# ZhengkunTian/Speech-Tranformer-Pytorch

Hardware: AMD Instinct MI355X
Metric: frames/sec/step (80-d fbank, 6+6L d256) at 1/2/4/8 MI355X vs CPU ref (higher is better)
Workload: dtype bf16; 1 GPU; BASELINE config 2: 6+6L d256 h4 dff1024 V4337, 80-d fbank, global B=32 split 32 per GPU (strong scaling, SURVEY 8e), T<=1000 (24060 valid frames on rank 0), L<=50; fwd+CE+bwd+clip+Adam (rate 0: weights held), dropout off; global_batch=32, parallelism=dp1, launch=hipGraph replay of the whole step, wire=fp32, dp_bucket_mb=8, nccl_algo=default, nccl_proto=default

## Files before the change

speech-tranformer-pytorch_amd/csrc/st_attn.hip:

```cpp
#include "st_attn_common.cuh"

int st_attn64_fwd_launch(hipStream_t stream, const void* args, int grid_x, int drop, int kpre);
int st_attn_xs_fwd_launch(hipStream_t stream, const void* args, int grid_x, int drop, const void* f1, const void* self);
void st_attn_xs_self_args(void* out, const void* Q, const void* K, const void* V, int ld, void* O, void* Ores, int ldo,
                          float* lse, const unsigned* drop_seed, unsigned drop_salt, int drop_thresh, float drop_scale);
int st_attn_xs_self_args_size();
void st_attn_xs_f1_args(void* out, const void* A, int lda, const void* R, int ldr, const void* wfrag, int n_blocks,
                        int next_blocks, float eps, const float* bo, const float* g0, const float* be0, void* out0,
                        void* xhat0, float* rstd0, const float* bq, void* Qout, int ldq);
int st_attn_xs_f1_args_size();
int st_attn_xs_tile_rows();
int st_attn_bwd64_launch(hipStream_t stream, const void* a, const void* ak, int n_q, int n_k, int drop);

namespace {

template <int DK, bool DROP, int KS, bool PS>
__global__ __launch_bounds__(256, (KS > 1 || DK > 64) ? 1 : 2) void attn_fwd_kernel(AttnArgs a) {
  using G = TileGeo<DK, TILE * KS>;
  constexpr int NT = DK / 16;
  constexpr int ND = DK / 32;
  constexpr int ROWS = TILE * KS, QROWS = WG_ROWS / KS;
  __shared__ __attribute__((aligned(16))) bf16 smem[4 * G::E];

  int b, h, tile;
// ... 500 lines not shown
  static const int n = [] {
    int dev = 0, cus = 0;
    if (hipGetDevice(&dev) != hipSuccess || hipDeviceGetAttribute(&cus, hipDeviceAttributeMultiprocessorCount, dev) != hipSuccess || cus <= 0) cus = 256;
    return cus;
  }();
  return n;
}
long long xsplit_bytes(int items, int xs, int d_k) { return (long long)XS_TICKETS * 4 + (long long)items * xs * 64 * d_k * 4; }

int plan(AttnArgs& a, const int* work, int n_work, int B, int H, int max_rows, int wg_rows = WG_ROWS) {
  a.work = work;
  a.H = H;
  a.tiles_max = (max_rows + wg_rows - 1) / wg_rows;
  return (work ? n_work : B * a.tiles_max) * H;
}

int attn_impl() {
  static const int v = [] { const char* e = getenv("ST_ATTN_IMPL"); return e ? atoi(e) : 0; }();
  return v;
}

struct AttnEnv {
  bool fwd64_off, xs_off;
  int bwd64;
};
AttnEnv read_attn_env() {
  auto off = [](const char* name) { const char* e = getenv(name); return e && e[0] == '0'; };
  const char* b = getenv("ST_ATTN_BWD64");
  return {off("ST_ATTN_FWD64"), off("ST_ATTN_XS"), (b && b[0] == '0') ? 1 : (b && b[0] == 'e') ? 2 : 0};
}
AttnEnv& attn_env() {
  static AttnEnv e = read_attn_env();
  return e;
}

bool fwd_long64(int d_k, int max_q, int max_k, int causal) {
  return d_k == 64 && !causal && max_q > 128 && attn_impl() != 1 && !attn_env().fwd64_off;
}

bool bwd_long64(int d_k, int max_q, int max_k, int causal, bool drop) {
  if (!(d_k == 64 && !causal && max_q > 128 && max_k > 128 && attn_impl() != 1)) return false;
  const int mode = attn_env().bwd64;
  return mode == 0 || (mode == 2 && !drop);
}

bool fwd_xs(int d_k, int max_q, int max_k, int causal) {
  return d_k == 64 && key_split(max_q, max_k, causal) && attn_impl() != 1 && !attn_env().xs_off;
}

}

extern "C" int st_env_refresh(void) {
  attn_env() = read_attn_env();
  return 0;
}

extern "C" int st_attn_tile_rows(int which, int d_k, int max_q, int max_k, int causal) {
  if (which == 0 && fwd_xs(d_k, max_q, max_k, causal)) return st_attn_xs_tile_rows();
  return WG_ROWS;
}

extern "C" int st_attn_fwd(hipStream_t stream, const void* Q, int ldq, const void* K, int ldk, const void* V, int ldv,
                           void* O, int ldo, void* Ores, float* lse, const int* q_off, const int* q_len, const int* k_off,
                           const int* k_len, int B, int H, int d_k, int max_q, int max_k, int q_rows_total, int causal,
                           float scale, const int* work, int n_work, const unsigned* drop_seed, unsigned drop_salt,
                           int drop_thresh, float drop_scale, int k_prescaled) {
  if (B <= 0 || H <= 0 || max_q <= 0 || (work && n_work <= 0)) return 0;
  int rc = check_common(d_k, ldq, ldk, ldv);
  if (rc) return rc;
  if (ldo & 7) return -3;
  if (B > 32767) return -4;
  AttnArgs a = {};
  a.Q = (const bf16*)Q; a.ldq = ldq; a.K = (const bf16*)K; a.ldk = ldk; a.V = (const bf16*)V; a.ldv = ldv;
  a.O = (bf16*)O; a.ldo = ldo; a.Ores = (bf16*)Ores; a.lse = lse; a.q_off = q_off; a.q_len = q_len; a.k_off = k_off; a.k_len = k_len;
  a.q_rows_total = q_rows_total; a.causal = causal; set_score_scales(a, scale, k_prescaled);
  const bool drop = set_drop(a, drop_seed, drop_salt, drop_thresh, drop_scale);
  a.psplit = (Ores != nullptr && max_q <= 64) ? 1 : 0;
  if (fwd_long64(d_k, max_q, max_k, causal)) {
    dim3 grid(plan(a, work, n_work, B, H, max_q));
    return st_attn64_fwd_launch(stream, &a, (int)grid.x, drop ? 1 : 0, k_prescaled ? 1 : 0);
  }
  const bool ks2 = key_split(max_q, max_k, causal);
  if (fwd_xs(d_k, max_q, max_k, causal))
    return st_attn_xs_fwd_launch(stream, &a, plan(a, work, n_work, B, H, max_q, st_attn_xs_tile_rows()), drop ? 1 : 0, nullptr, nullptr);
  dim3 grid(plan(a, work, n_work, B, H, max_q)), block(256);
#define ST_FWD(DKK, DR) \
  do { if (ks2 && a.psplit) hipLaunchKernelGGL((attn_fwd_kernel<DKK, DR, 2, true>), grid, block, 0, stream, a); \
       else if (ks2) hipLaunchKernelGGL((attn_fwd_kernel<DKK, DR, 2, false>), grid, block, 0, stream, a); \
       else if (a.psplit) hipLaunchKernelGGL((attn_fwd_kernel<DKK, DR, 1, true>), grid, block, 0, stream, a); \
       else hipLaunchKernelGGL((attn_fwd_kernel<DKK, DR, 1, false>), grid, block, 0, stream, a); } while (0)
  if (d_k == 64 && !drop) ST_FWD(64, false);
  else if (d_k == 64) ST_FWD(64, true);
  else if (d_k == 128 && !drop) ST_FWD(128, false);
  else if (d_k == 128) ST_FWD(128, true);
  else if (!drop) ST_FWD(32, false);
  else ST_FWD(32, true);
#undef ST_FWD
  ST_CHECK_LAUNCH();
  return 0;
}

extern "C" int st_attn_f1_applicable(int d_model, int d_k, int max_q, int max_k) {
  return (d_model == 256 && fwd_xs(d_k, max_q, max_k, 0)) ? 1 : 0;
}

namespace {
// ... 145 lines not shown
```

speech-tranformer-pytorch_amd/csrc/st_common.cuh:

```cuda
#pragma once

#ifdef ST_MERGE_FENCE
#define ST_PUBLISH_FENCE() __builtin_amdgcn_fence(__ATOMIC_RELEASE, "agent")
#define ST_MERGER_FENCE() __builtin_amdgcn_fence(__ATOMIC_ACQUIRE, "agent")
#else
#define ST_PUBLISH_FENCE() __builtin_amdgcn_fence(__ATOMIC_RELEASE, "wavefront")
#define ST_MERGER_FENCE() ((void)0)
#endif
#include <hip/hip_runtime.h>
#include <stdint.h>
#include "st_hip.h"

typedef __bf16 bf16;
typedef __bf16 bf16x8 __attribute__((ext_vector_type(8)));
typedef __bf16 bf16x4 __attribute__((ext_vector_type(4)));
typedef __bf16 bf16x2 __attribute__((ext_vector_type(2)));
typedef float f32x16 __attribute__((ext_vector_type(16)));
typedef float f32x4 __attribute__((ext_vector_type(4)));
typedef float f32x2 __attribute__((ext_vector_type(2)));

#define ST_WAVE 64
#define ST_LDS __attribute__((address_space(3)))

#define ST_CHECK_LAUNCH()                         \
  do {                                            \
    hipError_t e__ = hipGetLastError();           \
    if (e__ != hipSuccess) return (int)e__;       \
  } while (0)

__device__ __forceinline__ f32x16 mfma32(bf16x8 a, bf16x8 b, f32x16 c) {
  return __builtin_amdgcn_mfma_f32_32x32x16_bf16(a, b, c, 0, 0, 0);
}

__device__ __forceinline__ f32x16 zero16() {
  f32x16 z;
#pragma unroll
  for (int i = 0; i < 16; ++i) z[i] = 0.f;
  return z;
}

__device__ __forceinline__ bf16x8 zero_bf8() {
  bf16x8 z;
#pragma unroll
  for (int i = 0; i < 8; ++i) z[i] = (bf16)0.f;
  return z;
}

__device__ __forceinline__ int acc_row(int r, int hi) { return (r & 3) + 8 * (r >> 2) + 4 * hi; }

__device__ __forceinline__ bf16x8 gload8(const bf16* p, bool ok) {
  if (ok) return *reinterpret_cast<const bf16x8*>(p);
  return zero_bf8();
}

__device__ __forceinline__ bf16x8 frag_nat(const bf16* tile, int stride, int row, int c0) {
  return *reinterpret_cast<const bf16x8*>(tile + row * stride + c0);
}

__device__ __forceinline__ bf16x8 frag_tr(const bf16* tile, int stride, int row0, int ca, int cb) {
  const int l = threadIdx.x & 63;
  const int t = l & 15;
  const int colblk = ((l >> 4) & 1) * 16;
  const bf16* pa = tile + (ca + (t >> 2)) * stride + row0 + colblk + 4 * (t & 3);
  const bf16* pb = tile + (cb + (t >> 2)) * stride + row0 + colblk + 4 * (t & 3);
  bf16x4 lo = __builtin_amdgcn_ds_read_tr16_b64_v4bf16((ST_LDS bf16x4*)(pa));
  bf16x4 hi = __builtin_amdgcn_ds_read_tr16_b64_v4bf16((ST_LDS bf16x4*)(pb));
  bf16x8 f;
  f[0] = lo[0]; f[1] = lo[1]; f[2] = lo[2]; f[3] = lo[3];
  f[4] = hi[0]; f[5] = hi[1]; f[6] = hi[2]; f[7] = hi[3];
  return f;
}

__device__ __forceinline__ bf16x8 pack_acc8(const f32x16& a, int r0) {
  bf16x8 f;
#pragma unroll
// ... 68 lines not shown
```

speech-tranformer-pytorch_amd/csrc/st_gemm_sym.hip:

```cpp
#include "st_common.cuh"

#ifndef ST_GEMM_SC1
#define ST_GEMM_SC1 0
#endif
namespace {

#ifndef ST_GEMM_BK
#define ST_GEMM_BK 64
#endif
#ifndef ST_GEMM_OCC
#define ST_GEMM_OCC 2
#endif
constexpr int BK = ST_GEMM_BK;
constexpr int NS = BK + 8;
constexpr int CS_CM = 128;
constexpr int TILE_E = (128 * NS > BK * CS_CM) ? 128 * NS : BK * CS_CM;
constexpr int CH = BK / 16;
constexpr int CPR = BK / 8;

__device__ __attribute__((aligned(16))) float g_zero_f32[4];

enum Epi { EPI_BF16 = 0, EPI_BF16_RELU = 1, EPI_F32 = 2, EPI_BF16_MASK = 3, EPI_BF16_ADD = 4, EPI_F32_ATOMIC = 5,
           EPI_F32_ATOMIC_T = 6, EPI_BF16_DELTA = 7 };

// ... 468 lines not shown
}
}

extern "C" int st_wgrad_group(hipStream_t stream, int n, const void* const* X, const int* ldx, const void* const* dY,
                              const int* lddy, float* const* dW, const int* lddw, float* const* db, const int* tokens,
                              const int* K_in, const int* N_out, const int* splits) {
  for (int base = 0; base < n; base += GROUP_MAX) {
    GroupArgs g;
    g.n = 0;
    g.first[0] = 0;
    for (int q = base; q < n && q < base + GROUP_MAX; ++q) {
      if (tokens[q] <= 0 || K_in[q] <= 0 || N_out[q] <= 0) continue;
      if ((ldx[q] & 7) || (lddy[q] & 7) || (N_out[q] & 3)) return -1;
      if (ldx[q] < ((K_in[q] + 7) & ~7) || lddy[q] < ((N_out[q] + 7) & ~7)) return -3;
      GemmArgs a;
      a.M = K_in[q]; a.N = N_out[q]; a.Kc = tokens[q];
      plan_splits(a, splits[q] < 1 ? 1 : splits[q]);
      const int grid = a.splits * a.tiles_i * a.tiles_j;
      GroupProblem& p = g.p[g.n];
      p.X = (const bf16*)X[q]; p.ldx = ldx[q]; p.Y = (const bf16*)dY[q]; p.ldy = lddy[q]; p.D = dW[q]; p.ldd = lddw[q];
      p.bias = db ? db[q] : nullptr; p.M = a.M; p.N = a.N; p.Kc = a.Kc; p.c_per_split = a.c_per_split;
      p.tiles_i = a.tiles_i; p.tiles_j = a.tiles_j; p.splits = a.splits;
      g.first[g.n + 1] = g.first[g.n] + grid;
      ++g.n;
    }
    if (g.n == 0) continue;
    hipLaunchKernelGGL(gemm_wgrad_group_kernel, dim3(g.first[g.n]), dim3(256), 0, stream, g);
    ST_CHECK_LAUNCH();
  }
  return 0;
}

namespace {
int gemm_impl(hipStream_t stream, int x_cmajor, int y_cmajor, const void* X, int ldx, const void* Y,
              int ldy, void* D, int ldd, int M, int N, int Kc, float* bias, const void* aux,
              int ldaux, int epi, int splits, const unsigned* drop_seed, unsigned drop_salt,
              int drop_thresh, float drop_scale, int y_block_rows, long y_block_stride,
              long bias_block_stride, const void* aux2, void* split_work = nullptr, long long split_bytes = 0, int cs_lo = 0,
              int cs_hi = 0, float cs = 1.f) {
  if (M <= 0 || N <= 0 || Kc <= 0) return 0;
  int yseg_shift = 31;
  if (y_block_rows > 0) {
    if (y_block_rows < 128 || (y_block_rows & (y_block_rows - 1)) || x_cmajor || (y_block_stride & 7) ||
        (bias_block_stride & 3)) return -7;
    if (epi == EPI_F32_ATOMIC || epi == EPI_F32_ATOMIC_T || epi == EPI_BF16_DELTA) return -7;
    yseg_shift = __builtin_ctz(y_block_rows);
  }
  if ((ldx & 7) || (ldy & 7) || (N & 3) || epi < 0 || epi > 7) return -1;
  if (x_cmajor && !y_cmajor) return -2;
  if ((x_cmajor && ldx < ((M + 7) & ~7)) || (y_cmajor && ldy < ((N + 7) & ~7))) return -3;
  if (epi != EPI_F32 && epi != EPI_F32_ATOMIC && epi != EPI_F32_ATOMIC_T && ((ldd & 7) || (N & 7))) return -4;
  if ((epi == EPI_BF16_MASK || epi == EPI_BF16_ADD || epi == EPI_BF16_DELTA) && (ldaux & 7)) return -5;
  if (epi == EPI_BF16_DELTA && (!bias || !aux || (splits != 32 && splits != 64 && splits != 128) || (N % splits))) return -6;
  GemmArgs a;
  a.head_dim = epi == EPI_BF16_DELTA ? splits : 0;
  if (splits < 1) splits = 1;
  if (epi != EPI_F32_ATOMIC && epi != EPI_F32_ATOMIC_T && !(epi == EPI_BF16 && split_work)) splits = 1;
  a.split_ws = nullptr; a.split_tickets = nullptr;
  a.cs_lo = cs_lo; a.cs_hi = cs_hi; a.cs = cs;
  a.X = (const bf16*)X; a.ldx = ldx; a.Y = (const bf16*)Y; a.ldy = ldy; a.D = D; a.ldd = ldd;
  a.M = M; a.N = N; a.Kc = Kc; a.bias = bias; a.aux = (const bf16*)aux; a.ldaux = ldaux;
  a.aux2 = epi == EPI_BF16_DELTA ? (const bf16*)aux2 : nullptr;
  a.yseg_shift = yseg_shift;
  a.yseg_extra = y_block_rows > 0 ? y_block_stride - (long)y_block_rows * ldy : 0;
  a.bias_extra = y_block_rows > 0 ? bias_block_stride - (long)y_block_rows : 0;
  const bool drop = epi == EPI_BF16_RELU && drop_seed != nullptr && drop_thresh > 0;
  a.drop.seed = drop ? drop_seed : nullptr; a.drop.salt = drop_salt; a.drop.thresh = drop ? drop_thresh : 0;
  a.drop.scale = (drop || epi == EPI_BF16_MASK) && drop_scale > 0.f ? drop_scale : 1.f;
  dim3 grid(plan_splits(a, splits));
  if (epi == EPI_BF16 && a.splits > 1) {
    const long long tiles = (long long)a.tiles_i * a.tiles_j;
    if (tiles > 1024 || split_bytes < 4096 + tiles * a.splits * (256 * 64 * 4)) return -8;
    a.split_tickets = (unsigned*)split_work;
    a.split_ws = (float*)split_work + 1024;
  }
  int rc;
  if (!x_cmajor && !y_cmajor) rc = launch<false, false>(stream, a, epi, grid);
  else if (!x_cmajor && y_cmajor) rc = launch<false, true>(stream, a, epi, grid);
  else rc = launch<true, true>(stream, a, epi, grid);
  if (rc) return rc;
  ST_CHECK_LAUNCH();
  return 0;
}

}

extern "C" int st_gemm_splitk(hipStream_t stream, int y_cmajor, const void* X, int ldx, const void* Y, int ldy, void* D, int ldd,
                              int M, int N, int Kc, int splits, void* work, long long work_bytes) {
  if (!work || splits < 1) return -1;
  return gemm_impl(stream, 0, y_cmajor, X, ldx, Y, ldy, D, ldd, M, N, Kc, nullptr, nullptr, 0, EPI_BF16, splits, nullptr, 0u, 0, 1.f,
                   0, 0, 0, nullptr, work, work_bytes);
}

extern "C" int st_gemm_kscale(hipStream_t stream, const void* X, int ldx, const void* Y, int ldy, void* D, int ldd, int M, int N,
                              int Kc, float* bias, int col_lo, int col_hi, float scale) {
  if ((col_lo & 31) || (col_hi & 31) || col_lo < 0 || col_hi < col_lo || col_hi > N) return -9;
  return gemm_impl(stream, 0, 0, X, ldx, Y, ldy, D, ldd, M, N, Kc, bias, nullptr, 0, EPI_BF16, 1, nullptr, 0u, 0, 1.f, 0, 0, 0, nullptr,
                   nullptr, 0, col_lo, col_hi, scale);
}

extern "C" int st_gemm_stacked(hipStream_t stream, int x_cmajor, int y_cmajor, const void* X, int ldx, const void* Y,
                               int ldy, void* D, int ldd, int M, int N, int Kc, float* bias, const void* aux,
                               int ldaux, int epi, int splits, const unsigned* drop_seed, unsigned drop_salt,
                               int drop_thresh, float drop_scale, int y_block_rows, long y_block_stride,
                               long bias_block_stride) {
  return gemm_impl(stream, x_cmajor, y_cmajor, X, ldx, Y, ldy, D, ldd, M, N, Kc, bias, aux, ldaux, epi, splits, drop_seed,
// ... 11 lines not shown
```

speech-tranformer-pytorch_amd/csrc/st_rowchain.hip:

```cpp
#include "st_rowchain_common.cuh"
#include "st_rowchain_pipe.cuh"
#include "st_rowchain_pipe512.cuh"
#include <cstdlib>
#include <type_traits>

namespace {

extern __shared__ __attribute__((aligned(16))) float chain_vecs[];
__device__ __forceinline__ const float* chain_vec_src(const ChainArgs& a, int u) {
  if (u < 6) return u == 0 ? a.bo : u == 1 ? a.g0 : u == 2 ? a.be0 : u == 3 ? a.b2 : u == 4 ? a.g1 : a.be1;
  if (u < 6 + a.nc) return a.b1 ? a.b1 + (u - 6) * 256 : nullptr;
  return a.bp ? a.bp + (u - 6 - a.nc) * 256 : nullptr;
}
struct VecStage {
  f32x4 v[4];
  __device__ __forceinline__ void load(const ChainArgs& a, int wave, int l, int u0) {
    const int n = 6 + a.nc + a.nb;
#pragma unroll
    for (int i = 0; i < 4; ++i) {
      const int u = u0 + wave + 8 * i;
      const float* src = u < n ? chain_vec_src(a, u) : nullptr;
      v[i] = src ? *reinterpret_cast<const f32x4*>(src + 4 * l) : f32x4{0.f, 0.f, 0.f, 0.f};
    }
  }
// ... 712 lines not shown
      tile_store(c, ro, fa);
      if (a.Ores) tile_store(c, rr_, fb);
      __syncthreads();
      {
        const int row = c.r;
        float part_ = 0.f;
#pragma unroll
        for (int g = 0; g < 4; ++g) {
          const int at = row * AS + c.wave * 32 + 8 * g + 4 * c.hi;
          const bf16x4 o4 = *reinterpret_cast<const bf16x4*>(fa + at);
          bf16x4 r4 = {(bf16)0.f, (bf16)0.f, (bf16)0.f, (bf16)0.f};
          if (a.Ores) r4 = *reinterpret_cast<const bf16x4*>(fb + at);
          bf16x4 o;
#pragma unroll
          for (int e = 0; e < 4; ++e) {
            o[e] = (bf16)acc[0][4 * g + e];
            part_ += (float)o[e] * ((float)o4[e] + (float)r4[e]);
          }
          *reinterpret_cast<bf16x4*>(cur + at) = o;
        }
        part_ += wave_xor32(part_);
        if (c.hi == 0) red[0][c.wave * 32 + c.r] = part_;
      }
      __syncthreads();
      tile_out(c, cur, a.dctx, a.lddc);
      for (int i = c.tid; i < 4 * RB; i += 512) {
        const int h = i / RB, row = i % RB;
        if (row < c.nvalid) a.delta[(size_t)h * a.M + c.row0 + row] = red[0][(2 * h) * 32 + row] + red[0][(2 * h + 1) * 32 + row];
      }
    }
  }
  {
    int tsum = 0;
#pragma unroll
    for (int t = 0; t < TOUCH; ++t) tsum ^= touched[t];
    if (tsum == 0x5a5a5a5a && a.M < 0) red[0][0] = 1.f;
  }
}
}

namespace {
int row_tiles(int M) {
  static const int force = [] { const char* e = getenv("ST_CHAIN_MT"); return e ? atoi(e) : 0; }();
  if (force >= 1 && force <= 3) return force;
  const int cost[4] = {0, 27, 41, 59};
  int best = 1, best_cost = 1 << 30;
  for (int mt = 1; mt <= 3; ++mt) {
    const int tiles = (M + 32 * mt - 1) / (32 * mt), c = ((tiles + 255) / 256) * cost[mt];
    if (c < best_cost) { best = mt; best_cost = c; }
  }
  return best;
}
}

namespace {
int split_parts_for(int blocks, int nc) {
  if (nc < 2 || nc > 8 || blocks > 128) return 0;
  for (int p = nc; p >= 2; --p)
    if (nc % p == 0 && blocks * p <= 256) return p;
  return 0;
}
}

extern "C" int st_row_chain_mask_words(int M, int d_ff) {
  if (M <= 0 || d_ff <= 0) return 0;
  const int mt = row_tiles(M);
  return ((M + 32 * mt - 1) / (32 * mt)) * (d_ff / 256) * NW * 64;
}

extern "C" int st_row_chain(hipStream_t stream, int M, const void* wfrag, int n_blocks, int next_blocks, float eps, const void* A, int lda,
                            const void* R, int ldr, const float* bo, const float* g0, const float* be0, void* out0, void* xhat0,
                            float* rstd0, int d_ff, const float* b1, const float* b2, const float* g1, const float* be1, void* H,
                            unsigned long long* relu_bits, void* out1, void* xhat1, float* rstd1, const unsigned* drop_seed, unsigned drop1_salt,
                            int drop1_thresh, float drop1_scale, unsigned drop2_salt, int drop2_thresh, float drop2_scale,
                            int post_blocks, const float* bp, void* P, int ldp, void* split_work, long long split_bytes,
                            float post_kscale) {
  if (M <= 0) return 0;
  const bool pre = R != nullptr, ffn = d_ff > 0, post = post_blocks > 0;
  if (!A || !wfrag || (lda & 7) || (!pre && !ffn && !post)) return -1;
  if (pre && ((ldr & 7) || !bo || !g0 || !be0)) return -2;
  if (ffn && ((d_ff & 255) || !b1 || !b2 || !g1 || !be1 || !out1)) return -3;
  if (post && (!bp || !P || (ldp & 7) || ldp < 256 * post_blocks)) return -4;
  if (n_blocks != (pre ? 1 : 0) + (ffn ? 2 * (d_ff / 256) : 0) + post_blocks) return -5;
  ChainArgs a;
  a.M = M; a.wfrag = (const bf16x8*)wfrag; a.wave_frags = n_blocks * 16 + DEPTH; a.eps = eps;
  a.next_frags = next_blocks > 0 ? next_blocks * 16 + DEPTH : 0;
  a.A = (const bf16*)A; a.lda = lda; a.R = (const bf16*)R; a.ldr = ldr; a.bo = bo; a.g0 = g0; a.be0 = be0;
  a.out0 = (bf16*)out0; a.xhat0 = (bf16*)xhat0; a.rstd0 = rstd0;
  a.nc = d_ff / 256; a.b1 = b1; a.b2 = b2; a.g1 = g1; a.be1 = be1; a.H = (bf16*)H; a.relu_bits = relu_bits; a.out1 = (bf16*)out1; a.xhat1 = (bf16*)xhat1;
  a.rstd1 = rstd1;
  const bool on1 = ffn && drop_seed && drop1_thresh > 0, on2 = ffn && drop_seed && drop2_thresh > 0;
  a.drop1.seed = on1 ? drop_seed : nullptr; a.drop1.salt = drop1_salt; a.drop1.thresh = on1 ? drop1_thresh : 0;
  a.drop1.scale = on1 ? drop1_scale : 1.f;
  a.drop2.seed = on2 ? drop_seed : nullptr; a.drop2.salt = drop2_salt; a.drop2.thresh = on2 ? drop2_thresh : 0;
  a.drop2.scale = on2 ? drop2_scale : 1.f;
  a.nb = post_blocks; a.bp = bp; a.P = (bf16*)P; a.ldp = ldp;
  a.post_kscale = (post_blocks == 3 && post_kscale > 0.f) ? post_kscale : 1.f;
  const int mt = row_tiles(M);
  const dim3 grid((M + 32 * mt - 1) / (32 * mt)), blk(512);
  const bool drop = on1 || on2;
  a.split_ws = nullptr; a.split_tickets = nullptr; a.split_parts = 0;
  const int sp = split_parts_for((int)grid.x, a.nc);
  if (split_work && ffn && mt == 1 && sp >= 2) {
    const size_t words = (size_t)grid.x * sp * 512 * 16;
    if (split_bytes < (long long)((256 + words) * 4)) return -6;
    a.split_tickets = (unsigned*)split_work;
// ... 318 lines not shown
```

speech-tranformer-pytorch_amd/st_amd/chains.py:

```python
from __future__ import annotations

import math
from typing import List, Sequence, Tuple

import os
import torch

from . import native as nv
from . import rng

BLK = 256
BF16, F32 = torch.bfloat16, torch.float32


class Chain:
    __slots__ = ("stream", "n_blocks", "blocks", "next_blocks", "split_work")

    def __init__(self, stream, n_blocks, blocks, next_blocks=0):
        self.stream, self.n_blocks, self.blocks, self.next_blocks = stream, n_blocks, blocks, next_blocks
        self.split_work = None


def blocks_of(w: torch.Tensor, order: str = "rows") -> List[Tuple[torch.Tensor, int, int]]:
    n, k = w.shape
# ... 314 lines not shown
            a, f = SubPre(), SubPre()
            a.qkv, a.drop, a.kpre = qkv, sa._drop(dev), kpre
            a.ctx, a.lse, a.ores = EZ(M, d, rows), E(H * M, dt=F32), (EZ(M, d, rows) if need_bwd else None)
            nv.attn_fwd(qkv[:, :d], qkv[:, d:2 * d], qkv[:, 2 * d:], a.ctx, a.lse, rows.off, rows.len, rows.off, rows.len,
                        H, rows.max_len, False, scale, work=work, drop=a.drop, max_k=rows.max_len, ores=a.ores, k_prescaled=kpre)
            a.out, f.out, f.h = E(M, d), E(M, d), E(M, ff._st.d_ff)
            if need_bwd:
                a.xhat, a.rstd, f.xhat, f.rstd = E(M, d), E(M, dt=F32), E(M, d), E(M, dt=F32)
            f.drop1, f.drop2 = ff._drops(dev)
            if need_bwd and self.use_bwd:
                f.bits = torch.empty(nv.chain_mask_words(M, ff._st.d_ff, d), dtype=torch.int64, device=dev)
            nxt = layers[l + 1].slf_attn._st if l + 1 < n else None
            qkv = E(M, 3 * d) if nxt is not None else None
            nv.row_chain(a.ctx, self.e[l], pre=(x, sa._st.b_o, sa._st.gamma, sa._st.beta, a.out, a.xhat, a.rstd),
                         ffn=(ff._st.d_ff, ff._st.b1, ff._st.b2, ff._st.gamma, ff._st.beta, f.h, f.out, f.xhat, f.rstd, f.drop1,
                              f.drop2, f.bits),
                         post=(3 * d // BLK, nxt.b_qkv, qkv) if nxt is not None else None, post_kscale=kscale)
            x = f.out
            pres.append((a, f))
        if need_bwd and self.use_bwd:
            cb = EncoderBackward(self, list(layers), pres)
            for l, (a, f) in enumerate(pres):
                a.bwd = f.bwd = cb
                a.key, f.key = ("self", l), ("ffn", l)
        return x, pres


class DecoderChains:

    def __init__(self, layers, arena):
        self.arena = arena
        self.set = ChainSet(arena.device)
        f1, f2 = [], []
        n = len(layers)
        for l, layer in enumerate(layers):
            sa, ca, ff = layer.slf_attn._st, layer.enc_attn._st, layer.pos_ffn._st
            f1.append(self.set.add(blocks_of(sa.w_o) + blocks_of(ca.w_q)))
            nxt = blocks_of(layers[l + 1].slf_attn._st.w_qkv) if l + 1 < n else []
            f2.append(self.set.add(blocks_of(ca.w_o) + ffn_blocks(ff.w1, ff.w2) + nxt))
        self.set.finalize()
        self.f1 = [self.set.chain(c, True) for c in f1]
        self.f2 = [self.set.chain(c, True) for c in f2]
        if self.f2 and os.environ.get("ST_CHAIN_SPLIT", "1") != "0":
            work = torch.zeros(nv.split_work_words(), dtype=torch.int32, device=self.f2[0].stream.device)
            for ch in self.f2:
                ch.split_work = work
        self.bset = ChainSet(arena.device)
        b1, b2 = {}, {}
        for l in range(n - 1, -1, -1):
            sa, ca, ff = layers[l].slf_attn._st, layers[l].enc_attn._st, layers[l].pos_ffn._st
            head = t_blocks(blocks_of(layers[l + 1].slf_attn._st.w_qkv)) if l + 1 < n else []
            b2[l] = self.bset.add(head + ffn_blocks_bwd(ff.w1, ff.w2) + t_blocks(blocks_of(ca.w_o)))
            b1[l] = self.bset.add(t_blocks(blocks_of(ca.w_q)) + t_blocks(blocks_of(sa.w_o)))
        self.bset.finalize()
        self.bwd2 = [self.bset.chain(b2[l], True) for l in range(n)]
        if self.f2 and self.f2[0].split_work is not None and os.environ.get("ST_CHAIN_SPLIT", "1") != "f":
            for ch in self.bwd2:
                ch.split_work = self.f2[0].split_work
        self.bwd1 = [self.bset.chain(b1[l], True) for l in range(n)]
        self.use_bwd = sa.n_head * 64 == BLK
        self.layer_hook = None
        ChainHub.of(arena).add(self.set, self.bset)

    @staticmethod
    def plan(layers, arena):
        if not layers:
            return None
        for layer in layers:
            sa, ca, ff = layer.slf_attn, layer.enc_attn, layer.pos_ffn
            if any(getattr(m, "_st_arena", None) is not arena for m in (sa, ca, ff)):
                return None
            if sa._st.d_model != BLK or ff._st.d_ff % BLK:
                return None
        return DecoderChains(layers, arena)

    def forward(self, layers, x, kv, t_rows, in_rows, need_bwd: bool):
        from .functional import attn_work, rows_buffer
        M, d = x.shape
        dev = x.device

        def E(*shape, dt=BF16):
            return torch.empty(*shape, dtype=dt, device=dev)

        def EZ(m, n, layout):
            return rows_buffer(m, n, layout, dev)

        s0 = layers[0].slf_attn._st
        H = s0.n_head
        scale = 1.0 / math.sqrt(d // H)
        work_self, work_cross = attn_work(t_rows, t_rows, True, d // H, H)[0], attn_work(t_rows, in_rows, False, d // H, H)[0]
        qkv = E(M, 3 * d)
        nv.gemm(x, s0.w_qkv, qkv, bias=s0.b_qkv)
        pres = []
        n = len(layers)
        for l, layer in enumerate(layers):
            sa, ca, ff = layer.slf_attn, layer.enc_attn, layer.pos_ffn
            a, b, f = SubPre(), SubPre(), SubPre()
            a.qkv, a.drop = qkv, sa._drop(dev)
            a.ctx, a.lse, a.ores = EZ(M, d, t_rows), E(H * M, dt=F32), (EZ(M, d, t_rows) if need_bwd else None)
            a.out = EZ(M, d, t_rows)
            if need_bwd:
                a.xhat = EZ(M, d, t_rows)
                a.rstd = E(M, dt=F32) if t_rows.dense else torch.zeros(M, dtype=F32, device=dev)
            b.qkv = EZ(M, d, t_rows)
            b.kvbuf, b.drop = kv[:, l * 2 * d:(l + 1) * 2 * d], ca._drop(dev)
            b.ctx, b.lse, b.ores = EZ(M, d, t_rows), E(H * M, dt=F32), (EZ(M, d, t_rows) if need_bwd else None)
            nv.attn_sf1_fwd(qkv, a.ctx, a.lse, (x, sa._st.b_o, sa._st.gamma, sa._st.beta, a.out, a.xhat, a.rstd),
# ... 24 lines not shown
```

speech-tranformer-pytorch_amd/st_amd/functional.py:

```python
from __future__ import annotations

import collections
import math
import os
from typing import Optional

import torch
import torch.nn as nn

from . import native as nv

BF16, F32, I32 = torch.bfloat16, torch.float32, torch.int32
LN_EPS = 1e-6


_ROWS_CACHE = {}


class Rows:

    __slots__ = ("B", "off", "len", "max_len", "total", "_pos", "lens_host", "dense", "_scatter", "_work", "_seq", "valid_rows")

    def __init__(self, off, length, max_len, total, lens_host=None, dense=True):
        self.dense = dense
# ... 324 lines not shown
    return nv.gemm_splitk(dY, W, out, max(2, min(6, 128 // tiles)), y_cmajor=True)


def _empty(rows, cols, like, dtype=BF16):
    return torch.empty(rows, cols, dtype=dtype, device=like.device)


class TailBuffers:
    active = None
    N_MAX = 256

    def __init__(self):
        self.mode, self.specs, self.bufs, self.i, self.table, self.missed = "record", [], [], 0, None, 0

    def request(self, m, n, layout, device):
        if self.mode == "record":
            self.specs.append((int(m), int(n), layout))
            return torch.zeros(m, n, dtype=BF16, device=device)
        if self.i < len(self.bufs) and self.specs[self.i][:2] == (int(m), int(n)) and self.specs[self.i][2] is layout:
            self.i += 1
            return self.bufs[self.i - 1]
        self.missed += 1
        return torch.zeros(m, n, dtype=BF16, device=device)

    def materialize(self, device):
        self.specs = self.specs[:TailBuffers.N_MAX]
        self.bufs = [torch.zeros(m, n, dtype=BF16, device=device) for m, n, _ in self.specs]
        rows = []
        for buf, (m, n, layout) in zip(self.bufs, self.specs):
            rows += [buf.data_ptr(), n * buf.element_size(), m, layout.valid_rows.data_ptr()]
        rows += [0, 0, 0, 0] * (TailBuffers.N_MAX - len(self.bufs))
        self.table = torch.tensor(rows, dtype=torch.int64).to(device)
        self.mode, self.i = "serve", 0
        return self


def rows_buffer(m, n, layout, device):
    if layout.dense:
        return torch.empty(m, n, dtype=BF16, device=device)
    tb = TailBuffers.active
    if tb is not None and layout._seq is not None and n * 2 % 16 == 0:
        return tb.request(m, n, layout, device)
    return torch.zeros(m, n, dtype=BF16, device=device)


class CrossGradAcc:
    __slots__ = ("n", "seen", "buf")

    def __init__(self, n: int):
        self.n, self.seen, self.buf = n, 0, None


class CrossKv:
    __slots__ = ("mods", "n", "w_stride", "b_stride", "seen", "dkv")

    def __init__(self, mods, w_stride, b_stride):
        self.mods, self.n, self.w_stride, self.b_stride, self.seen, self.dkv = mods, len(mods), w_stride, b_stride, 0, None

    @staticmethod
    def plan(mods):
        if len(mods) < 2:
            return None
        a = mods[0]._st_arena
        if a is None or a._grad_ready_cb is not None:
            return None
        cached = getattr(mods[0], "_st_crosskv", None)
        if cached is None or cached[0] is not a:
            cached = (a, CrossKv._strides(mods, a))
            mods[0]._st_crosskv = cached
        return None if cached[1] is None else CrossKv(list(mods), *cached[1])

    @staticmethod
    def _strides(mods, a):
        if any(m._st_arena is not a for m in mods):
            return None
        d = mods[0]._st.d_model
        if any(m._st.d_model != d or m._st.n_head != mods[0]._st.n_head for m in mods) or (2 * d) & (2 * d - 1) or d < 64:
            return None
        w_off = [a.offset[id(m.linear_k.weight)] for m in mods]
        b_off = [a.offset[id(m.linear_k.bias)] for m in mods]
        ws, bs = w_off[1] - w_off[0], b_off[1] - b_off[0]
        if ws <= 0 or bs <= 0 or any(w_off[i + 1] - w_off[i] != ws or b_off[i + 1] - b_off[i] != bs for i in range(len(mods) - 1)):
            return None
        return ws, bs


class CrossKvSlot:
    __slots__ = ("state", "idx")

    def __init__(self, state, idx):
        self.state, self.idx = state, idx


class CrossKvFn(torch.autograd.Function):
    @staticmethod
    def forward(ctx, enc, anchor, state: CrossKv):
        s0 = state.mods[0]._st
        kv = _empty(enc.shape[0], state.n * 2 * s0.d_model, enc)
        linear_fwd(enc, s0.w_kv, kv, s0.b_kv, stack=(state.n, state.w_stride, state.b_stride))
        ctx.save_for_backward(enc)
        ctx.state = state
        return kv

    @staticmethod
    def backward(ctx, dkv):
        enc, = ctx.saved_tensors
        state = ctx.state
        s0 = state.mods[0]._st
        w = 2 * s0.d_model
        dkv = dkv.contiguous()
        for l, m in enumerate(state.mods):
            s = m._st
            m._st_arena.attach_grads(s.params, s.lo, s.hi)
            wgrad(dkv[:, l * w:(l + 1) * w], enc, s.g_w_kv, gB=s.g_b_kv)
        d_enc = _empty(enc.shape[0], s0.d_model, enc)
        nv.gemm(dkv, s0.w_kv, d_enc, y_cmajor=True, stack=(state.n, state.w_stride, 0))
        return d_enc, None, None


class LnLink:
    __slots__ = ("ok", "st", "arena", "xhat", "rstd", "g_bias", "drop", "ds")

    def __init__(self):
        self.ok, self.ds = False, None

    def offer(self, mod, xhat, rstd, g_bias, drop=None):
        self.ok, self.st, self.arena, self.xhat, self.rstd, self.g_bias = True, mod._st, mod._st_arena, xhat, rstd, g_bias
        self.drop = drop

    def fused_dgrad(self, dY, W, aux):
        st = self.st
        self.arena.attach_grads(st.params, st.lo, st.hi)
        ds = _empty(dY.shape[0], W.shape[1], dY)
        nv.gemm_lnbwd(dY, W, aux, self.xhat, self.rstd, st.gamma, ds, st.g_gamma, st.g_beta, self.g_bias, drop=self.drop)
        self.ds = ds
        return ds

    def claim(self, dout):
        ds, self.ds = self.ds, None
        if ds is None:
            return None
        if dout.data_ptr() != ds.data_ptr() or dout.shape != ds.shape:
            raise RuntimeError("LnLink: the gradient reaching this sublayer is not the one its consumer fused the "
                               "LayerNorm backward into (its output has more than one consumer?)")
        return ds


def _input_grad(link, dY, W, aux):
    if link is not None and link.ok:
        return link.fused_dgrad(dY, W, aux)
    dx = _empty(dY.shape[0], W.shape[1], dY)
    dgrad(dY, W, dx, epi=nv.EPI_BF16_ADD, aux=aux)
    return dx


class CtcPlan:

    def __init__(self, targets, target_lengths, input_lengths, in_rows: Rows, blank: int, v_pad: int):
        dev = targets.device
        B, L = targets.shape
        self.B, self.L, self.C, self.T = B, L, L + 1, in_rows.max_len
        self.blank = int(blank)
        self._tl = target_lengths.to(device=dev, dtype=torch.int64)
        self._il = input_lengths.to(device=dev, dtype=torch.int64)
        self.classes = torch.zeros(B, L, dtype=torch.int64, device=dev)
        self.cols = torch.zeros(B, L + 1, dtype=I32, device=dev)
        self.scat = torch.zeros(B, L + 1, dtype=I32, device=dev)
        self.finite = torch.zeros(B, dtype=torch.bool, device=dev)
        self.tl = self._tl.clamp_min(1)
# ... 615 lines not shown
```

speech-tranformer-pytorch_amd/st_amd/native.py:

```python
from __future__ import annotations

import ctypes
import os
import re
from typing import Optional

import torch

from . import build as _build

_CTYPES = {"int": ctypes.c_int, "unsigned": ctypes.c_uint, "float": ctypes.c_float, "long": ctypes.c_long,
           "long long": ctypes.c_longlong}


def _argtypes(name: str, params: str):
    argtypes = []
    for param in ([] if params.strip() == "void" else params.split(",")):
        words = param.replace("const", " ").split()
        ctype = ctypes.c_void_p if "*" in param or words[0] == "st_stream_t" else _CTYPES.get(" ".join(words[:-1]))
        if ctype is None:
            raise RuntimeError("include/st_hip.h: %s: parameter '%s' has a type the binding does not know" % (name, param.strip()))
        argtypes.append(ctype)
    return argtypes

# ... 256 lines not shown
        if not 0.0 <= p < 1.0:
            raise ValueError("Drop: p must be in [0, 1)")
        self.seed, self.salt = seed, int(salt) & 0xFFFFFFFF
        self.thresh = min(255, int(round(256.0 * p)))
        self.scale = 256.0 / (256 - self.thresh)

    @property
    def p_effective(self) -> float:
        return self.thresh / 256.0


def _drop(d: Optional["Drop"]):
    if d is None or d.thresh == 0:
        return None, 0, 0, 1.0
    return d.seed.data_ptr(), d.salt, d.thresh, d.scale


def gemm(X, Y, out, bias=None, aux=None, epi=EPI_BF16, x_cmajor=False, y_cmajor=False, splits=1,
         m=None, n=None, kc=None, drop=None, delta=None, head_dim=0, stack=None, aux2=None):
    _mat(X, BF16, "X"), _mat(Y, BF16, "Y")
    _mat(out, F32 if epi in (EPI_F32, EPI_F32_ATOMIC, EPI_F32_ATOMIC_T) else BF16, "out")
    M = m if m is not None else (X.shape[1] if x_cmajor else X.shape[0])
    N = n if n is not None else (Y.shape[1] if y_cmajor else Y.shape[0])
    Kc = kc if kc is not None else (X.shape[0] if x_cmajor else X.shape[1])
    blocks, block_rows, y_stride, b_stride = 1, 0, 0, 0
    if stack is not None:
        blocks, y_stride, b_stride = stack
        block_rows = Y.shape[0]
        if y_cmajor:
            Kc = blocks * block_rows
        else:
            N = blocks * block_rows
    need = (N, M) if epi == EPI_F32_ATOMIC_T else (M, N)
    if out.shape[0] < need[0] or out.shape[1] < need[1]:
        raise ValueError("gemm: out %s too small for %dx%d" % (tuple(out.shape), need[0], need[1]))
    _vec(bias, F32, N // blocks if not y_cmajor else N, "bias")
    if epi == EPI_BF16_DELTA:
        if head_dim not in (32, 64, 128) or N % head_dim:
            raise ValueError("gemm: EPI_BF16_DELTA needs head_dim in {32, 64, 128} dividing N")
        _vec(delta, F32, (N // head_dim) * M, "delta")
        bias, splits = delta, head_dim
    ldaux = 0
    if epi in (EPI_BF16_MASK, EPI_BF16_ADD, EPI_BF16_DELTA):
        _mat(aux, BF16, "aux")
        ldaux = aux.stride(0)
        if aux2 is not None:
            _mat(aux2, BF16, "aux2")
            if epi != EPI_BF16_DELTA or aux2.stride(0) != ldaux or aux2.shape != aux.shape:
                raise ValueError("gemm: aux2 goes with EPI_BF16_DELTA and must have aux's shape and stride")
    esz = 4 if epi in (EPI_F32, EPI_F32_ATOMIC, EPI_F32_ATOMIC_T) else 2
    _tag("gemm", int(x_cmajor), int(y_cmajor), M, N, Kc, epi,
         io=(2.0 * M * Kc, 2.0 * N * Kc, float(esz) * M * N, 2.0 * M * N if aux is not None else 0, 2.0 * M * N if aux2 is not None else 0))
    dropargs = _drop(drop) if epi in (EPI_BF16_RELU, EPI_BF16_MASK) else _drop(None)
    if stack is None:
        rc = load().st_gemm(_stream(), int(x_cmajor), int(y_cmajor), X.data_ptr(), X.stride(0), Y.data_ptr(),
                            Y.stride(0), out.data_ptr(), out.stride(0), M, N, Kc, _p(bias), _p(aux), ldaux, epi, splits,
                            *dropargs, _p(aux2))
    else:
        rc = load().st_gemm_stacked(_stream(), int(x_cmajor), int(y_cmajor), X.data_ptr(), X.stride(0), Y.data_ptr(),
                                    Y.stride(0), out.data_ptr(), out.stride(0), M, N, Kc, _p(bias), _p(aux), ldaux,
                                    epi, splits, *dropargs, block_rows, y_stride, b_stride)
    _check(rc, "st_gemm")
    return out


def gemm_ws(X, W, out, bias=None, relu=False, drop=None, stack=None):
    _mat(X, BF16, "X"), _mat(W, BF16, "W"), _mat(out, BF16, "out")
    M, K = X.shape
    N = W.shape[0]
    blocks, block_rows, w_stride, b_stride = 1, 0, 0, 0
    if stack is not None:
        blocks, w_stride, b_stride = stack
        block_rows = W.shape[0]
        N = blocks * block_rows
    if out.shape[0] < M or out.shape[1] < N:
        raise ValueError("gemm_ws: out %s too small for %dx%d" % (tuple(out.shape), M, N))
    _vec(bias, F32, N // blocks, "bias")
    _tag("gemm", 0, 0, M, N, K, EPI_BF16_RELU if relu else EPI_BF16, io=(2.0 * M * K, 2.0 * N * K, 2.0 * M * N))
    rc = load().st_gemm_ws(_stream(), X.data_ptr(), X.stride(0), W.data_ptr(), W.stride(0), out.data_ptr(), out.stride(0),
                           M, N, K, _p(bias), int(relu), *(_drop(drop) if relu else _drop(None)), block_rows, w_stride, b_stride)
    _check(rc, "st_gemm_ws")
    return out


def gemm_kscale(X, W, out, bias, col_lo, col_hi, scale):
    _mat(X, BF16, "X"), _mat(W, BF16, "W"), _mat(out, BF16, "out")
    M, K = X.shape
    N = W.shape[0]
    _vec(bias, F32, N, "bias")
    _tag("gemm", 0, 0, M, N, K, EPI_BF16, io=(2.0 * M * K, 2.0 * N * K, 2.0 * M * N, 0, 0))
    _check(load().st_gemm_kscale(_stream(), X.data_ptr(), X.stride(0), W.data_ptr(), W.stride(0), out.data_ptr(), out.stride(0),
                                 M, N, K, _p(bias), int(col_lo), int(col_hi), float(scale)), "st_gemm_kscale")
    return out


def ws_ok(M, N, K):
    return K == 256 and N % 256 == 0 and M >= 12288


def wgrad_group(problems, wide=False):
    problems = list(problems)
    n = len(problems)
    if n == 0:
        return
    PA, IA = ctypes.c_void_p * n, ctypes.c_int * n
    X, dY, dW, dB = PA(), PA(), PA(), PA()
# ... 940 lines not shown
```

speech-tranformer-pytorch_amd/transformer/Models.py:

```python
import torch
import torch.nn as nn

import transformer.Constants as Constants
from st_amd import functional as F_
from st_amd import rng
from st_amd.arena import arena_of, bundle
from st_amd.chains import DecoderChains, EncoderChains
from transformer.Embedding import PositionalEncoding
from transformer.Layers import EncoderLayer, DecoderLayer


def _check_lengths(lengths, limit, what):
    if int(lengths.min()) < 1:
        raise ValueError("%s: every utterance needs length >= 1 (a fully masked softmax row is NaN in the reference)" % what)
    if int(lengths.max()) > limit:
        raise ValueError("%s: length %d exceeds the positional-encoding table (%d)" % (what, int(lengths.max()), limit))


class Encoder(nn.Module):

    def __init__(self, input_size, n_max_seq, n_layers=6, n_head=8, d_k=64, d_v=64,
                 d_model=512, d_inner_hid=1024, dropout=0.1, emb_scale=1):
        super(Encoder, self).__init__()
        self.n_max_seq, self.d_model, self.emb_scale = n_max_seq, d_model, emb_scale
# ... 48 lines not shown
        hit = getattr(self, "_st_chains", None)
        if hit is None or hit[0] is not arena:
            ec = EncoderChains.plan(list(self.layer_stack), arena) if self.use_row_chains else None
            hit = (arena, ec)
            self._st_chains = hit
        return hit[1] if self.use_row_chains else None

    def forward(self, inputs, inputs_length, return_attns=False):
        if not return_attns:
            e, rows = self.forward_rows(inputs, inputs_length)
            return F_.UnpackFn.apply(e, rows, inputs.shape[1]), []
        T = inputs.shape[1]
        with F_.AttnTap() as tap:
            e, rows = self.forward_rows(inputs, inputs_length)
        return F_.UnpackFn.apply(e, rows, T), [tap.of(layer.slf_attn, T, T)[0] for layer in self.layer_stack]


class Decoder(nn.Module):

    def __init__(self, vocab_size, n_max_seq, n_layers=6, n_head=8, d_k=64, d_v=64,
                 d_model=512, d_inner_hid=1024, dropout=0.1, emb_scale=1):
        super(Decoder, self).__init__()
        self.n_max_seq, self.output_dim, self.d_model, self.emb_scale = n_max_seq, vocab_size, d_model, emb_scale
        self.position_enc = PositionalEncoding(dropout, d_model, self.n_max_seq)
        self.tgt_word_emb = nn.Embedding(vocab_size, d_model, Constants.PAD)
        self.layer_stack = nn.ModuleList([
            DecoderLayer(d_model, d_inner_hid, n_head, d_k, d_v, dropout=dropout) for _ in range(n_layers)])
        self.use_row_chains = True

    def _st_bind(self, a):
        emb = self.tgt_word_emb.weight
        lo, hi = a.span([emb])
        return bundle(d_model=self.d_model, pad_idx=Constants.PAD, emb_params=[emb], emb_lo=lo, emb_hi=hi,
                      emb=a.master(emb), g_emb=a.grad_view(emb), pe=self.position_enc.pe[0])

    def row_chains(self, arena):
        hit = getattr(self, "_st_chains", None)
        if hit is None or hit[0] is not arena:
            dc = DecoderChains.plan(list(self.layer_stack), arena) if self.use_row_chains else None
            hit = (arena, dc)
            self._st_chains = hit
        return hit[1] if self.use_row_chains else None

    def forward_rows(self, tokens, tgt_len, enc_rows_mat, in_rows, t_rows=None):
        _check_lengths(tgt_len, min(self.n_max_seq, tokens.shape[1]), "Decoder")
        arena = arena_of(self)
        with arena.scope():
            if t_rows is None:
                t_rows = F_.Rows.packed(tgt_len, tokens.device)
            y = F_.EmbedFn.apply(self.tgt_word_emb.weight, self, tokens.contiguous(), t_rows)
            link = None
            ckv = F_.CrossKv.plan([layer.enc_attn for layer in self.layer_stack])
            if ckv is not None:
                kv = F_.CrossKvFn.apply(enc_rows_mat, self.layer_stack[0].enc_attn.linear_k.weight, ckv)
                dc = self.row_chains(arena)
                pres = None
                if dc is not None:
                    need_bwd = torch.is_grad_enabled() and (y.requires_grad or kv.requires_grad)
                    with torch.no_grad():
                        y_out, pres = dc.forward(self.layer_stack, y, kv, t_rows, in_rows, need_bwd)
                    if not need_bwd:
                        F_.AttnTap.record_chain(self.layer_stack, pres, t_rows, in_rows)
                        return y_out, t_rows
                for l, layer in enumerate(self.layer_stack):
                    y, link = layer.forward_rows(y, kv, t_rows, in_rows, F_.CrossKvSlot(ckv, l), link,
                                                 pre=pres[l] if pres is not None else None)
            else:
                acc = F_.CrossGradAcc(len(self.layer_stack)) if enc_rows_mat.requires_grad else None
                for layer in self.layer_stack:
                    y, link = layer.forward_rows(y, enc_rows_mat, t_rows, in_rows, acc, link)
        return y, t_rows

    def forward(self, outputs_data, outputs_pos, input_pos, enc_output, return_attns=False):
        in_rows = F_.Rows.packed(input_pos, enc_output.device)
        enc = F_.PackFn.apply(enc_output.float(), in_rows)
        if not return_attns:
            y, t_rows = self.forward_rows(outputs_data, outputs_pos, enc, in_rows)
            return F_.UnpackFn.apply(y, t_rows, outputs_data.shape[1]), [], []
        L, T = outputs_data.shape[1], enc_output.shape[1]
        with F_.AttnTap() as tap:
            y, t_rows = self.forward_rows(outputs_data, outputs_pos, enc, in_rows)
        return (F_.UnpackFn.apply(y, t_rows, L), [tap.of(layer.slf_attn, L, L)[0] for layer in self.layer_stack],
                [tap.of(layer.enc_attn, L, T)[0] for layer in self.layer_stack])


class Transformer(nn.Module):

    def __init__(self, config):
        super(Transformer, self).__init__()

        def need(*names):
            for n in names:
                v = getattr(config, n, None) if not isinstance(config, dict) else config.get(n)
                if v is not None:
                    return v
            raise KeyError("Transformer(config): missing required key %s" % "/".join(names))

        def opt(name, default):
            v = getattr(config, name, None) if not isinstance(config, dict) else config.get(name)
            return default if v is None else v

        self.return_attns = opt('return_attns', None)
        common = dict(n_head=need('n_heads'), d_k=need('d_k'), d_v=need('d_v'), d_model=need('d_model'),
                      d_inner_hid=need('d_inner_hid'), dropout=need('dropout'), emb_scale=opt('emb_scale', 1))
        self.vocab_size, self.d_model = need('vocab_size'), common['d_model']
        self._d_k, self._n_head = common['d_k'], common['n_head']
        self.encoder = Encoder(input_size=need('feature_dim'), n_max_seq=need('max_inputs_length', 'max_input_length'),
                               n_layers=need('num_enc_layer'), **common)
# ... 78 lines not shown
```

Measured before the change: 8.948 million frames/s.

## Route cross-attention KV dgrad through a row-chain GEMM with pre-fragmented weights

Adds a dedicated row-tiled GEMM kernel for the stacked cross-attention K/V input-gradient (N=256). It uses pre-packed MFMA weight fragments held in a register ring and double-buffers X tiles in LDS, reusing the row-chain pipeline machinery. The kernel is meant to replace the generic stacked gemm for large M (default at least 2048 rows), which is the encoder output across 6 decoder layers. It adds a new fragment chain to the block set and new env knobs, and falls back to the old path when its preconditions fail.

Result: no change. 8.995 million frames/s (median of 6 runs) (+0.5%).

```diff
diff --git a/speech-tranformer-pytorch_amd/csrc/st_attn.hip b/speech-tranformer-pytorch_amd/csrc/st_attn.hip
--- a/speech-tranformer-pytorch_amd/csrc/st_attn.hip
+++ b/speech-tranformer-pytorch_amd/csrc/st_attn.hip
@@ -576,6 +576,7 @@
 
 extern "C" int st_env_refresh(void) {
   attn_env() = read_attn_env();
+  st_host::gemm_env_refresh();
   return 0;
 }
 
diff --git a/speech-tranformer-pytorch_amd/csrc/st_common.cuh b/speech-tranformer-pytorch_amd/csrc/st_common.cuh
--- a/speech-tranformer-pytorch_amd/csrc/st_common.cuh
+++ b/speech-tranformer-pytorch_amd/csrc/st_common.cuh
@@ -21,6 +21,11 @@
 
 #define ST_WAVE 64
 #define ST_LDS __attribute__((address_space(3)))
+
+namespace st_host {
+bool gemm_rows_launch(hipStream_t stream, const void* X, int ldx, const void* wfrag, int n_blocks, void* D, int ldd, int M);
+void gemm_env_refresh();
+}
 
 #define ST_CHECK_LAUNCH()                         \
   do {                                            \
diff --git a/speech-tranformer-pytorch_amd/csrc/st_gemm_rows.cuh b/speech-tranformer-pytorch_amd/csrc/st_gemm_rows.cuh
--- /dev/null
+++ b/speech-tranformer-pytorch_amd/csrc/st_gemm_rows.cuh
@@ -0,0 +1,118 @@
+#pragma once
+#include "st_rowchain_pipe.cuh"
+
+namespace {
+
+struct GemmRowsArgs {
+  int M, nb;
+  const bf16x8* wfrag; int wave_frags;
+  const bf16* X; int ldx;
+  bf16* D; int ldd;
+};
+
+template <int MT, bool ST, bool LD> struct StageSide {
+  const Ctx<MT>& c;
+  TileRegs<MT>& t;
+  bf16* dst;
+  const bf16* src;
+  int ld;
+  __device__ __forceinline__ void a(int) {}
+  __device__ __forceinline__ void b(int k2) {
+    if (k2 < 2 * MT) {
+      const int id = c.tid + k2 * 512, rr = id >> 5, cc = id & 31;
+      if (ST) *reinterpret_cast<bf16x8*>(dst + rr * AS + cc * 8) = t.v[k2];
+      if (LD) t.v[k2] = *reinterpret_cast<const bf16x8*>(src + (size_t)min(rr, c.nvalid - 1) * ld + cc * 8);
+    }
+  }
+};
+
+template <int MT>
+__global__ __launch_bounds__(512, 1) void gemm_rows_kernel(GemmRowsArgs a) {
+  constexpr int RB = 32 * MT, TE = RB * AS;
+  __shared__ __attribute__((aligned(16))) bf16 tiles[2 * TE];
+  Ctx<MT> c;
+  c.tid = threadIdx.x; c.wave = __builtin_amdgcn_readfirstlane(c.tid >> 6); c.l = c.tid & 63; c.hi = c.l >> 5; c.r = c.l & 31;
+  c.row0 = blockIdx.x * RB; c.nvalid = min(RB, a.M - c.row0);
+  const bf16x8* sbase = a.wfrag + (size_t)c.wave * a.wave_frags * 64;
+  auto blk = [&](int b) { return sbase + (size_t)b * 16 * 64; };
+  c.ws = sbase;
+#pragma unroll
+  for (int i = 0; i < 8; ++i) c.ring[i] = sbase[i * 64 + c.l];
+  const bf16* xrow = a.X + (size_t)c.row0 * a.ldx;
+  auto tile = [&](int b) { return tiles + (b & 1) * TE; };
+  const int nb = a.nb;
+
+  TileRegs<MT> tr;
+  NoSide ns;
+  {
+    TileRegs<MT> t0;
+    StageSide<MT, false, true> l0{c, t0, nullptr, xrow, a.ldx};
+#pragma unroll
+    for (int p = 0; p < 2 * MT; ++p) l0.b(p);
+    if (nb > 1) {
+      StageSide<MT, false, true> l1{c, tr, nullptr, xrow + 256, a.ldx};
+#pragma unroll
+      for (int p = 0; p < 2 * MT; ++p) l1.b(p);
+    }
+    tile_store(c, t0, tile(0));
+  }
+  __syncthreads();
+  f32x16 acc[MT];
+  zero_acc(acc);
+  int b = 0;
+  for (; b + 2 < nb; ++b) {
+    StageSide<MT, true, true> s{c, tr, tile(b + 1), xrow + (size_t)(b + 2) * 256, a.ldx};
+    block_mma_p(c, blk(b), blk(b + 1), tile(b), acc, s);
+    __syncthreads();
+  }
+  if (b + 1 < nb) {
+    StageSide<MT, true, false> s{c, tr, tile(b + 1), nullptr, 0};
+    block_mma_p(c, blk(b), blk(b + 1), tile(b), acc, s);
+    __syncthreads();
+    ++b;
+  }
+  block_mma_p(c, blk(b), blk(b + 1), tile(b), acc, ns);
+  __syncthreads();
+
+  bf16* ot = tiles;
+#pragma unroll
+  for (int mt = 0; mt < MT; ++mt)
+#pragma unroll
+    for (int g = 0; g < 4; ++g) {
+      bf16x4 o;
+#pragma unroll
+      for (int e = 0; e < 4; ++e) o[e] = (bf16)acc[mt][4 * g + e];
+      *reinterpret_cast<bf16x4*>(ot + (mt * 32 + c.r) * AS + c.wave * 32 + 8 * g + 4 * c.hi) = o;
+    }
+  __syncthreads();
+  tile_out(c, ot, a.D, a.ldd);
+}
+
+struct GemmRowsEnv { bool off; int min_rows, mt; };
+GemmRowsEnv read_gemm_rows_env() {
+  const char* o = getenv("ST_KV_DGRAD_ROWS");
+  const char* m = getenv("ST_KV_DGRAD_MIN_ROWS");
+  const char* t = getenv("ST_GEMM_ROWS_MT");
+  return {o && o[0] == '0', m && m[0] ? atoi(m) : 2048, t ? atoi(t) : 0};
+}
+GemmRowsEnv& gemm_rows_env() {
+  static GemmRowsEnv e = read_gemm_rows_env();
+  return e;
+}
+
+}
+
+void st_host::gemm_env_refresh() { gemm_rows_env() = read_gemm_rows_env(); }
+
+bool st_host::gemm_rows_launch(hipStream_t stream, const void* X, int ldx, const void* wfrag, int n_blocks, void* D, int ldd, int M) {
+  const GemmRowsEnv& env = gemm_rows_env();
+  if (env.off || !wfrag || n_blocks < 1 || M < env.min_rows || ldx < 256 * n_blocks || ldd < 256 || (ldx & 7) || (ldd & 7)) return false;
+  GemmRowsArgs a;
+  a.M = M; a.nb = n_blocks; a.wfrag = (const bf16x8*)wfrag; a.wave_frags = n_blocks * 16 + DEPTH;
+  a.X = (const bf16*)X; a.ldx = ldx; a.D = (bf16*)D; a.ldd = ldd;
+  const int mt = env.mt == 2 || env.mt == 3 ? env.mt : max(2, ::row_tiles(M));
+  const dim3 grid((M + 32 * mt - 1) / (32 * mt));
+  if (mt == 3) hipLaunchKernelGGL(gemm_rows_kernel<3>, grid, dim3(512), 0, stream, a);
+  else hipLaunchKernelGGL(gemm_rows_kernel<2>, grid, dim3(512), 0, stream, a);
+  return true;
+}
diff --git a/speech-tranformer-pytorch_amd/csrc/st_gemm_sym.hip b/speech-tranformer-pytorch_amd/csrc/st_gemm_sym.hip
--- a/speech-tranformer-pytorch_amd/csrc/st_gemm_sym.hip
+++ b/speech-tranformer-pytorch_amd/csrc/st_gemm_sym.hip
@@ -544,6 +544,11 @@
   if (epi != EPI_F32 && epi != EPI_F32_ATOMIC && epi != EPI_F32_ATOMIC_T && ((ldd & 7) || (N & 7))) return -4;
   if ((epi == EPI_BF16_MASK || epi == EPI_BF16_ADD || epi == EPI_BF16_DELTA) && (ldaux & 7)) return -5;
   if (epi == EPI_BF16_DELTA && (!bias || !aux || (splits != 32 && splits != 64 && splits != 128) || (N % splits))) return -6;
+  if (y_block_rows > 0 && !x_cmajor && y_cmajor && epi == EPI_BF16 && !bias && !split_work && aux && ldaux > 0 && N == 256 &&
+      Kc == 256 * ldaux && st_host::gemm_rows_launch(stream, X, ldx, aux, ldaux, D, ldd, M)) {
+    ST_CHECK_LAUNCH();
+    return 0;
+  }
   GemmArgs a;
   a.head_dim = epi == EPI_BF16_DELTA ? splits : 0;
   if (splits < 1) splits = 1;
diff --git a/speech-tranformer-pytorch_amd/csrc/st_rowchain.hip b/speech-tranformer-pytorch_amd/csrc/st_rowchain.hip
--- a/speech-tranformer-pytorch_amd/csrc/st_rowchain.hip
+++ b/speech-tranformer-pytorch_amd/csrc/st_rowchain.hip
@@ -788,6 +788,7 @@
   return best;
 }
 }
+#include "st_gemm_rows.cuh"
 
 namespace {
 int split_parts_for(int blocks, int nc) {
diff --git a/speech-tranformer-pytorch_amd/st_amd/chains.py b/speech-tranformer-pytorch_amd/st_amd/chains.py
--- a/speech-tranformer-pytorch_amd/st_amd/chains.py
+++ b/speech-tranformer-pytorch_amd/st_amd/chains.py
@@ -390,7 +390,9 @@
             head = t_blocks(blocks_of(layers[l + 1].slf_attn._st.w_qkv)) if l + 1 < n else []
             b2[l] = self.bset.add(head + ffn_blocks_bwd(ff.w1, ff.w2) + t_blocks(blocks_of(ca.w_o)))
             b1[l] = self.bset.add(t_blocks(blocks_of(ca.w_q)) + t_blocks(blocks_of(sa.w_o)))
+        kvd = self.bset.add([blk for layer in layers for blk in t_blocks(blocks_of(layer.enc_attn._st.w_kv))])
         self.bset.finalize()
+        self.kv_dgrad = self.bset.chain(kvd)
         self.bwd2 = [self.bset.chain(b2[l], True) for l in range(n)]
         if self.f2 and self.f2[0].split_work is not None and os.environ.get("ST_CHAIN_SPLIT", "1") != "f":
             for ch in self.bwd2:
diff --git a/speech-tranformer-pytorch_amd/st_amd/functional.py b/speech-tranformer-pytorch_amd/st_amd/functional.py
--- a/speech-tranformer-pytorch_amd/st_amd/functional.py
+++ b/speech-tranformer-pytorch_amd/st_amd/functional.py
@@ -400,10 +400,11 @@
 
 
 class CrossKv:
-    __slots__ = ("mods", "n", "w_stride", "b_stride", "seen", "dkv")
+    __slots__ = ("mods", "n", "w_stride", "b_stride", "seen", "dkv", "wfrag")
 
     def __init__(self, mods, w_stride, b_stride):
         self.mods, self.n, self.w_stride, self.b_stride, self.seen, self.dkv = mods, len(mods), w_stride, b_stride, 0, None
+        self.wfrag = None
 
     @staticmethod
     def plan(mods):
@@ -462,7 +463,8 @@
             m._st_arena.attach_grads(s.params, s.lo, s.hi)
             wgrad(dkv[:, l * w:(l + 1) * w], enc, s.g_w_kv, gB=s.g_b_kv)
         d_enc = _empty(enc.shape[0], s0.d_model, enc)
-        nv.gemm(dkv, s0.w_kv, d_enc, y_cmajor=True, stack=(state.n, state.w_stride, 0))
+        nv.gemm(dkv, s0.w_kv, d_enc, y_cmajor=True, stack=(state.n, state.w_stride, 0),
+                aux=state.wfrag.stream if state.wfrag is not None and s0.d_model == 256 else None)
         return d_enc, None, None
 
 
diff --git a/speech-tranformer-pytorch_amd/st_amd/native.py b/speech-tranformer-pytorch_amd/st_amd/native.py
--- a/speech-tranformer-pytorch_amd/st_amd/native.py
+++ b/speech-tranformer-pytorch_amd/st_amd/native.py
@@ -332,6 +332,12 @@
     _tag("gemm", int(x_cmajor), int(y_cmajor), M, N, Kc, epi,
          io=(2.0 * M * Kc, 2.0 * N * Kc, float(esz) * M * N, 2.0 * M * N if aux is not None else 0, 2.0 * M * N if aux2 is not None else 0))
     dropargs = _drop(drop) if epi in (EPI_BF16_RELU, EPI_BF16_MASK) else _drop(None)
+    if epi == EPI_BF16 and aux is not None:
+        if stack is None or not y_cmajor or x_cmajor or bias is not None or N != 256 or Kc % 256:
+            raise ValueError("gemm: with EPI_BF16, aux is the fragment stream of a stacked dgrad with 256 output columns and no bias")
+        if aux.dtype != BF16 or aux.dim() != 1 or not aux.is_cuda or aux.numel() != 8 * (Kc // 256 * 16 + wfrag_depth()) * 512:
+            raise ValueError("gemm: the fragment stream must be a 1-D bf16 GPU tensor of one chain with Kc / 256 blocks")
+        ldaux = Kc // 256
     if stack is None:
         rc = load().st_gemm(_stream(), int(x_cmajor), int(y_cmajor), X.data_ptr(), X.stride(0), Y.data_ptr(),
                             Y.stride(0), out.data_ptr(), out.stride(0), M, N, Kc, _p(bias), _p(aux), ldaux, epi, splits,
diff --git a/speech-tranformer-pytorch_amd/transformer/Models.py b/speech-tranformer-pytorch_amd/transformer/Models.py
--- a/speech-tranformer-pytorch_amd/transformer/Models.py
+++ b/speech-tranformer-pytorch_amd/transformer/Models.py
@@ -124,8 +124,9 @@
             link = None
             ckv = F_.CrossKv.plan([layer.enc_attn for layer in self.layer_stack])
             if ckv is not None:
+                dc = self.row_chains(arena)
+                ckv.wfrag = dc.kv_dgrad if dc is not None else None
                 kv = F_.CrossKvFn.apply(enc_rows_mat, self.layer_stack[0].enc_attn.linear_k.weight, ckv)
-                dc = self.row_chains(arena)
                 pres = None
                 if dc is not None:
                     need_bwd = torch.is_grad_enabled() and (y.requires_grad or kv.requires_grad)
```
